# stujen/fiveEqSCM

Hardware: AMD Instinct MI355X
Metric: ensemble_member_timesteps_per_sec (higher is better)
Workload: dtype f64

## Files before the change

fiveeqscm_amd/csrc/fiveeq_member.hpp:

```cpp
#pragma once

namespace fiveeq {

template <typename V>
__device__ __forceinline__ V gas_forcing(const KGas<typename Lane<V>::S>& kg, const V Cg) {
    using S = typename Lane<V>::S;
    const auto pos = fe_gt0(Cg);
    V Fg = kg.f2 * (Cg - kg.C0);
    if constexpr (Lane<V>::W == 1) {
        if (kg.f1 != S(0)) Fg = pos ? fe_fma(kg.f1, fe_log(pos ? Cg * kg.inv_C0 : S(1)), Fg) : Fg;
        if (kg.f3 != S(0)) Fg = fe_fma(kg.f3, (pos ? fe_sqrt(pos ? Cg : S(1)) : S(0)) - kg.sqrtC0, Fg);
    } else {
        if (kg.f1 != S(0)) Fg = fe_sel(pos, fma3<V>(kg.f1, fe_log(fe_sel(pos, Cg * kg.inv_C0, (V)S(1))), Fg), Fg);
        if (kg.f3 != S(0)) Fg = fma3<V>(kg.f3, fe_sel(pos, fe_sqrt(fe_sel(pos, Cg, (V)S(1))), (V)S(0)) - kg.sqrtC0, Fg);
    }
    return Fg;
}

template <typename V, typename L, int g, bool INV, bool COMP = false>
__device__ __forceinline__ V gas_step(const KModel<typename Lane<V>::S>& km, const KGas<typename Lane<V>::S>& kg,
                                      const typename Lane<V>::S* __restrict__ drv, const V (&rr)[3 * L::G], const V T_old,
                                      V (&R)[L::SP], V (&out)[L::G], V (&cum)[L::G], V (&Rlo)[L::SP]) {
    using S = typename Lane<V>::S;
    static_assert(!INV || Lane<V>::W == 1, "the concentration-driven form has no packed instantiation");
    static_assert(!COMP || (!INV && sizeof(S) == 4), "the compensated form is an fp32 form of the emission-driven step");
    constexpr int P = L::pools(g);
    constexpr int o = L::off(g);
    V sumR = R[o];
#pragma unroll
    for (int i = 1; i < P; ++i) sumR += R[o + i];
    const V G_a = sumR * kg.inv_c;
    V G_u;
    if constexpr (INV) G_u = cum[g] - G_a;
    else G_u = drv[3 + g] - G_a;
    V iirf = fma3<V>(kg.ra, G_a, fma3<V>(rr[3 * g + 2], T_old, fma3<V>(rr[3 * g + 1], G_u, rr[3 * g])));
    iirf = fe_min(iirf, km.iirf_max);
    const V alpha = kg.g0 * fe_exp(iirf * kg.inv_g1);
    const V inv_alpha = fe_rcp(alpha);
    V em1[P];
#pragma unroll
    for (int i = 0; i < P; ++i) em1[i] = fe_expm1_neg(kg.ndt_over_tau[i] * inv_alpha);
    V E;
    if constexpr (INV) {
        V num = V(0), den = V(0);
#pragma unroll
        for (int i = 0; i < P; ++i) {
            num += fe_fma(R[o + i], em1[i], R[o + i]);
            den = fe_fma(kg.atc[i], em1[i], den);
        }
        E = (num - (drv[g] - kg.C0)) / (alpha * den);
        cum[g] = fe_fma(E, km.dt, cum[g]);
        out[g] = E;
    } else {
        E = (V)drv[g];
    }
    const V Ea = E * alpha;
    V sumN = (V)S(0);
#pragma unroll
    for (int i = 0; i < P; ++i) {
        const V Ri = R[o + i];
        V Rn;
        if constexpr (COMP) {
            const V y = fe_fma(em1[i], fma3<V>(-kg.atc[i], Ea, Ri), Rlo[o + i]);
            Rn = Ri + y;
            Rlo[o + i] = y - (Rn - Ri);
        } else {
            Rn = fe_fma(em1[i], fma3<V>(-kg.atc[i], Ea, Ri), Ri);
        }
        R[o + i] = Rn;
        sumN += Rn;
    }
    const V Cg = kg.C0 + sumN;
    if constexpr (!INV) out[g] = Cg;
    if constexpr (COMP) {
        const auto pos = fe_gt0(Cg);
        V Fg = kg.f2 * sumN;
        if (kg.f1 != S(0)) {
            const V x = sumN * kg.inv_C0;
            const V u = fe_sel(pos, (V)S(1) + x, (V)S(1));
            const V lg = fe_log(u) + (x - (u - (V)S(1)));
            Fg = fe_sel(pos, fma3<V>(kg.f1, lg, Fg), Fg);
        }
        if (kg.f3 != S(0)) {
            const V den = fe_sqrt(fe_sel(pos, Cg, (V)S(1))) + kg.sqrtC0;
            Fg = fma3<V>(kg.f3, fe_sel(pos, sumN * fe_rcp(den), (V)(-kg.sqrtC0)), Fg);
        }
        return Fg;
    } else {
        return gas_forcing<V>(kg, Cg);
    }
}

constexpr int MAX_FEXT = 4;
template <typename V, typename L, bool INV, bool COMP, bool FORC = false>
__device__ __forceinline__ void member_step(const KModel<typename Lane<V>::S>& km, const typename Lane<V>::S* __restrict__ drv,
                                            const V (&rr)[3 * L::G], const V (&qq)[2],
                                            V (&R)[L::SP], V (&S)[2], V (&out)[L::G], V& Tnew, V (&cum)[L::G],
                                            V (&Rlo)[L::SP], const V* fs = nullptr, const int fs_stride = 1,
                                            const typename Lane<V>::S* xr = nullptr, const int n_fext = 0) {
    static_assert(!FORC || (!INV && !COMP), "the forcing scales are carried by the plain forward form only");
    const V T_old = S[0] + S[1];
    V F = (V)drv[6];
    if constexpr (FORC) {
#pragma unroll
        for (int k = 0; k < MAX_FEXT; ++k)
            if (k < n_fext) F = fma3<V>(fs[(L::G + k) * fs_stride], xr[k], F);
    }
    asm volatile("" ::: "memory");
    const V F0 = gas_step<V, L, 0, INV, COMP>(km, km.gas[0], drv, rr, T_old, R, out, cum, Rlo);
    if constexpr (FORC) F = fe_fma(fs[0 * fs_stride], F0, F);
    else F += F0;
    if constexpr (L::G > 1) {
        asm volatile("" ::: "memory");
        const V F1 = gas_step<V, L, 1, INV, COMP>(km, km.gas[1], drv, rr, T_old, R, out, cum, Rlo);
        if constexpr (FORC) F = fe_fma(fs[1 * fs_stride], F1, F);
        else F += F1;
    }
    if constexpr (L::G > 2) {
        asm volatile("" ::: "memory");
        const V F2 = gas_step<V, L, 2, INV, COMP>(km, km.gas[2], drv, rr, T_old, R, out, cum, Rlo);
        if constexpr (FORC) F = fe_fma(fs[2 * fs_stride], F2, F);
        else F += F2;
    }
#pragma unroll
    for (int j = 0; j < 2; ++j) S[j] = fma3<V>(km.em1_d[j], fe_fma(-qq[j], F, S[j]), S[j]);
    Tnew = S[0] + S[1];
}
template <typename V, typename L, bool INV = false>
__device__ __forceinline__ void member_step(const KModel<typename Lane<V>::S>& km, const typename Lane<V>::S* __restrict__ drv,
                                            const V (&rr)[3 * L::G], const V (&qq)[2],
                                            V (&R)[L::SP], V (&S)[2], V (&out)[L::G], V& Tnew, V (&cum)[L::G]) {
    V no_Rlo[L::SP];
    member_step<V, L, INV, false>(km, drv, rr, qq, R, S, out, Tnew, cum, no_Rlo);
}
template <typename V, typename L>
__device__ __forceinline__ void member_step(const KModel<typename Lane<V>::S>& km, const typename Lane<V>::S* __restrict__ drv,
                                            const V (&rr)[3 * L::G], const V (&qq)[2],
                                            V (&R)[L::SP], V (&S)[2], V (&C)[L::G], V& Tnew) {
    V unused[L::G];
    member_step<V, L, false>(km, drv, rr, qq, R, S, C, Tnew, unused);
}

__device__ __forceinline__ void misfit_update(const double o, const double p, const double b, const double Tw, double& A,
                                              double& U, double& Vq) {
    A = A + b * Tw;
    const double d = Tw - o;
    const double pd = p * d;
    U = U + pd;
    Vq = Vq + pd * d;
}
__device__ __forceinline__ double lane_member(const double v, int) { return v; }
__device__ __forceinline__ double lane_member(const float v, int) { return (double)v; }
__device__ __forceinline__ double lane_member(const float2v v, int j) { return (double)(j == 0 ? v.x : v.y); }

template <typename T>
__device__ __forceinline__ void stage_model(KModel<T>* dst) {
    constexpr int NW = sizeof(KModel<T>) / sizeof(T);
    const T* src = (const T*)__builtin_amdgcn_kernarg_segment_ptr();
    for (int i = threadIdx.x; i < NW; i += FIVEEQ_BLOCK) reinterpret_cast<T*>(dst)[i] = src[i];
}

template <typename V>
__device__ __forceinline__ V load_lane(const typename Lane<V>::S* p) { return *reinterpret_cast<const V*>(p); }
__device__ __forceinline__ void store_lane(double* p, double v, bool) { *p = v; }
__device__ __forceinline__ void store_lane(float* p, float v, bool) { *p = v; }
__device__ __forceinline__ void store_lane(float* p, float2v v, bool full) {
    if (full) *reinterpret_cast<float2v*>(p) = v;
    else *p = v.x;
}
template <typename V, bool NT>
__device__ __forceinline__ V load_row(const typename Lane<V>::S* p) {
    if constexpr (NT) return __builtin_nontemporal_load(reinterpret_cast<const V*>(p));
    else return load_lane<V>(p);
}
template <bool NT, typename S, typename V>
__device__ __forceinline__ void store_row(S* p, V v, bool full) {
    if constexpr (!NT) store_lane(p, v, full);
    else if constexpr (sizeof(V) == sizeof(S)) __builtin_nontemporal_store(v, p);
    else {
        if (full) __builtin_nontemporal_store(v, reinterpret_cast<V*>(p));
        else __builtin_nontemporal_store(v.x, p);
    }
}

template <typename V>
__device__ __forceinline__ void misfit_step(const double* ob, const V Tn, double* acc, const int64_t mem_stride,
                                            const int64_t word_stride, const bool full) {
    const double o_t = ob[0], p_t = ob[1], b_t = ob[2];
    if (p_t != 0.0 || b_t != 0.0) {
#pragma unroll
        for (int j = 0; j < Lane<V>::W; ++j) {
            if (j == 0 || full) {
                double* a = acc + j * mem_stride;
                double A = a[0], U = a[word_stride], Vq = a[2 * word_stride];
                misfit_update(o_t, p_t, b_t, lane_member(Tn, j), A, U, Vq);
                a[0] = A;
                a[word_stride] = U;
                a[2 * word_stride] = Vq;
            }
        }
    }
}

enum Park { PARK_FIRST, PARK_LAST };
struct LaneSpan {
    int64_t m;
    bool active, full;
    int64_t mm;
};
template <int W, int BLOCK, Park PARK>
__device__ __forceinline__ LaneSpan lane_span(const int64_t n) {
    const int64_t m = ((int64_t)blockIdx.x * BLOCK + threadIdx.x) * W;
    const bool active = m < n;
    const bool full = m + (W - 1) < n;
    const int64_t mm = active ? m : (PARK == PARK_LAST ? ((n - 1) & ~(int64_t)(W - 1)) : 0);
    return LaneSpan{m, active, full, mm};
}

}
```

fiveeqscm_amd/csrc/fiveeq_step.hpp:

```cpp
#pragma once

namespace fiveeq {


#ifdef FIVEEQ_STEP_WAVES
#define FIVEEQ_STEP_ATTR __attribute__((amdgpu_waves_per_eu(FIVEEQ_STEP_WAVES, FIVEEQ_STEP_WAVES)))
#else
#define FIVEEQ_STEP_ATTR
#endif
template <typename T>
struct UniformRows {
    uint32_t mask;
    T val[3 * MAX_GAS + 2];
};
template <typename V, int P0, int P1, int P2, bool BINS, bool NT, bool MISFIT, bool FORC, bool UNI>
__device__ __forceinline__ void step_body(
    const typename Lane<V>::S* __restrict__ drive, const int n_steps, const int t,
    const int64_t n, const int64_t ld,
    const typename Lane<V>::S* __restrict__ r, const typename Lane<V>::S* __restrict__ q,
    typename Lane<V>::S* __restrict__ R, typename Lane<V>::S* __restrict__ S,
    typename Lane<V>::S* __restrict__ C_traj, typename Lane<V>::S* __restrict__ T_traj,
    const int n_rows, double* __restrict__ stats,
    unsigned short* __restrict__ bin_ring, const int ring_rows,
    const double hist_lo, const double hist_inv_w, const int n_bins,
    const double* __restrict__ obs, double* __restrict__ misfit,
    const typename Lane<V>::S* __restrict__ fscale,
    const typename Lane<V>::S* __restrict__ fext, const int n_fext,
    const UniformRows<typename Lane<V>::S>& uni) {
    using L = Layout<P0, P1, P2>;
    using T = typename Lane<V>::S;
    constexpr int W = Lane<V>::W;
    constexpr bool NTT = true;
    static_assert(!FORC || (!BINS && !NT), "the forcing scales: no histogram ring, default row policy");
    static_assert(!UNI || (!BINS && !MISFIT && !FORC), "the single-valued rows: the plain forward form only");
    __shared__ T drv[DRIVE_STRIDE];
    const auto [m, active, full, mm] = lane_span<W, FIVEEQ_STEP_BLOCK, PARK_LAST>(n);
    __shared__ KModel<T> km_s;
    constexpr int NW = sizeof(KModel<T>) / sizeof(T);
    static_assert(NW <= FIVEEQ_STEP_BLOCK, "model must stage in one pass");
    const T* kargs = (const T*)__builtin_amdgcn_kernarg_segment_ptr();
    T stage_v = T(0), drv_v = T(0);
    if (threadIdx.x < NW) stage_v = kargs[threadIdx.x];
    if (threadIdx.x < DRIVE_STRIDE) drv_v = drive[(int64_t)t * DRIVE_STRIDE + threadIdx.x];
    const KModel<T>& kmr = km_s;

    V rr[3 * L::G], qq[2], Rv[L::SP], Sv[2], Cv[L::G];
#pragma unroll
    for (int k = 0; k < L::SP; ++k) Rv[k] = load_row<V, NT>(R + k * ld + mm);
#pragma unroll
    for (int k = 0; k < 2; ++k) Sv[k] = load_row<V, NT>(S + k * ld + mm);
    if constexpr (UNI) {
#pragma unroll
        for (int k = 0; k < 3 * L::G; ++k) {
            if (uni.mask & (1u << k)) rr[k] = (V)uni.val[k];
            else rr[k] = load_row<V, NT>(r + k * ld + mm);
        }
#pragma unroll
        for (int k = 0; k < 2; ++k) {
            if (uni.mask & (1u << (3 * L::G + k))) qq[k] = (V)uni.val[3 * L::G + k];
            else qq[k] = load_row<V, NT>(q + k * ld + mm);
        }
    } else {
#pragma unroll
        for (int k = 0; k < 3 * L::G; ++k) rr[k] = load_row<V, NT>(r + k * ld + mm);
#pragma unroll
        for (int k = 0; k < 2; ++k) qq[k] = load_row<V, NT>(q + k * ld + mm);
    }
    V fs[FORC ? L::G + MAX_FEXT : 1];
    if constexpr (FORC) {
#pragma unroll
        for (int k = 0; k < L::G + MAX_FEXT; ++k) fs[k] = k < L::G + n_fext ? load_row<V, NT>(fscale + k * ld + mm) : (V)T(0);
    }

    if (threadIdx.x < NW) reinterpret_cast<T*>(&km_s)[threadIdx.x] = stage_v;
    if (threadIdx.x < DRIVE_STRIDE) drv[threadIdx.x] = drv_v;
    __syncthreads();

    V Tn = (V)T(0);
    if constexpr (FORC) {
        V no_cum[L::G], no_Rlo[L::SP];
        member_step<V, L, false, false, true>(kmr, drv, rr, qq, Rv, Sv, Cv, Tn, no_cum, no_Rlo, fs, 1,
                                              fext + (int64_t)t * MAX_FEXT, n_fext);
    } else {
        member_step<V, L>(kmr, drv, rr, qq, Rv, Sv, Cv, Tn);
    }
    if (active) {
#pragma unroll
        for (int k = 0; k < L::SP; ++k) store_row<NT>(R + k * ld + m, Rv[k], full);
#pragma unroll
        for (int k = 0; k < 2; ++k) store_row<NT>(S + k * ld + m, Sv[k], full);
        const int row = __builtin_amdgcn_readfirstlane((int)drv[7]);
        if (row >= 0 && row < n_rows) {
            if (C_traj != nullptr) {
                T* c = C_traj + (int64_t)row * L::G * ld + m;
#pragma unroll
                for (int g = 0; g < L::G; ++g) store_row<NTT>(c + g * ld, Cv[g], full);
            }
            if (T_traj != nullptr) store_row<NTT>(T_traj + (int64_t)row * ld + m, Tn, full);
        }
        if constexpr (MISFIT) misfit_step(obs + (int64_t)t * 4, Tn, misfit + m, 1, ld, full);
        if constexpr (BINS)
            store_bin(bin_ring + (int64_t)(t % ring_rows) * ld + m, make_rule(T(0), hist_lo, hist_inv_w, n_bins), Tn, full);
    }
    if (stats != nullptr) {
        const int64_t n_rec = (n + 63) >> 6;
        const int64_t wave = (int64_t)blockIdx.x * (FIVEEQ_STEP_BLOCK / 64) + (threadIdx.x >> 6);
        if constexpr (W == 1) {
            if (wave < n_rec) wave_stats(active, Tn, stats + (wave * n_steps + t) * 4);
        } else {
            if (2 * wave < n_rec)
                wave_stats(active, full, Tn, stats + (2 * wave * n_steps + t) * 4,
                           2 * wave + 1 < n_rec ? stats + ((2 * wave + 1) * n_steps + t) * 4 : nullptr);
        }
    }
}

template <typename V, int P0, int P1, int P2, bool BINS = false, bool NT = false, bool MISFIT = false, bool FORC = false>
__global__ __launch_bounds__(FIVEEQ_STEP_BLOCK) FIVEEQ_STEP_ATTR void step_kernel(
    const KModel<typename Lane<V>::S> km, const typename Lane<V>::S* __restrict__ drive, const int n_steps, const int t,
    const int64_t n, const int64_t ld,
    const typename Lane<V>::S* __restrict__ r, const typename Lane<V>::S* __restrict__ q,
    typename Lane<V>::S* __restrict__ R, typename Lane<V>::S* __restrict__ S,
    typename Lane<V>::S* __restrict__ C_traj ,
    typename Lane<V>::S* __restrict__ T_traj ,
    const int n_rows, double* __restrict__ stats ,
    unsigned short* __restrict__ bin_ring , const int ring_rows,
    const double hist_lo, const double hist_inv_w, const int n_bins,
    const double* __restrict__ obs , double* __restrict__ misfit ,
    const typename Lane<V>::S* __restrict__ fscale ,
    const typename Lane<V>::S* __restrict__ fext , const int n_fext) {
    step_body<V, P0, P1, P2, BINS, NT, MISFIT, FORC, false>(drive, n_steps, t, n, ld, r, q, R, S, C_traj, T_traj, n_rows, stats,
                                                            bin_ring, ring_rows, hist_lo, hist_inv_w, n_bins, obs, misfit, fscale,
                                                            fext, n_fext, UniformRows<typename Lane<V>::S>{});
}

template <typename V, int P0, int P1, int P2, bool NT = false>
__global__ __launch_bounds__(FIVEEQ_STEP_BLOCK) FIVEEQ_STEP_ATTR void step_uniform_kernel(
    const KModel<typename Lane<V>::S> km, const typename Lane<V>::S* __restrict__ drive, const int n_steps, const int t,
    const int64_t n, const int64_t ld,
    const typename Lane<V>::S* __restrict__ r, const typename Lane<V>::S* __restrict__ q,
    typename Lane<V>::S* __restrict__ R, typename Lane<V>::S* __restrict__ S,
    typename Lane<V>::S* __restrict__ C_traj ,
    typename Lane<V>::S* __restrict__ T_traj ,
    const int n_rows, double* __restrict__ stats ,
    const UniformRows<typename Lane<V>::S> uni) {
    step_body<V, P0, P1, P2, false, NT, false, false, true>(drive, n_steps, t, n, ld, r, q, R, S, C_traj, T_traj, n_rows, stats,
                                                            nullptr, 0, 0.0, 0.0, 0, nullptr, nullptr, nullptr, nullptr, 0, uni);
}

template <typename U>
__global__ __launch_bounds__(FIVEEQ_BLOCK) void uniform_rows_kernel(const int64_t n, const int64_t ld, const int n_r,
                                                                    const U* __restrict__ rows_r, const U* __restrict__ rows_q,
                                                                    unsigned int* __restrict__ differs, U* __restrict__ first) {
    const int row = blockIdx.y;
    const U* p = row < n_r ? rows_r + (int64_t)row * ld : rows_q + (int64_t)(row - n_r) * ld;
    const U v0 = p[0];
    U diff = 0;
    for (int64_t i = (int64_t)blockIdx.x * FIVEEQ_BLOCK + threadIdx.x; i < n; i += (int64_t)gridDim.x * FIVEEQ_BLOCK)
        diff |= p[i] ^ v0;
    if (__ballot(diff != 0) != 0 && (threadIdx.x & 63) == 0) atomicOr(differs, 1u << row);
    if (blockIdx.x == 0 && threadIdx.x == 0) first[row] = v0;
}

template <typename V, typename L>
struct ScenForc {
    static constexpr bool FS_LDS = false;
};
template <>
struct ScenForc<double, Layout<4, 1, 1>> {
    static constexpr bool FS_LDS = true;
};
template <typename V, int P0, int P1, int P2, bool NT = false, bool FORC = false>
__global__ __launch_bounds__(FIVEEQ_STEP_BLOCK) FIVEEQ_STEP_ATTR void step_scen_kernel(
    const KModel<typename Lane<V>::S> km, const typename Lane<V>::S* __restrict__ drive, const int n_steps, const int t,
    const int64_t n, const int64_t ld, const int n_scen,
    const typename Lane<V>::S* __restrict__ r, const typename Lane<V>::S* __restrict__ q,
    typename Lane<V>::S* __restrict__ R, typename Lane<V>::S* __restrict__ S,
    typename Lane<V>::S* __restrict__ C_traj, typename Lane<V>::S* __restrict__ T_traj,
    const int n_rows, double* __restrict__ stats,
    const typename Lane<V>::S* __restrict__ fscale ,
    const typename Lane<V>::S* __restrict__ fext , const int n_fext) {
    using L = Layout<P0, P1, P2>;
    using T = typename Lane<V>::S;
    constexpr int W = Lane<V>::W;
    constexpr bool NTT = true;
    static_assert(!FORC || !NT, "the forcing scales: default row policy");
    constexpr bool FS_LDS = FORC && ScenForc<V, L>::FS_LDS;
    const auto [m, active, full, mm] = lane_span<W, FIVEEQ_STEP_BLOCK, PARK_LAST>(n);
    __shared__ KModel<T> km_s;
    constexpr int NW = sizeof(KModel<T>) / sizeof(T);
    static_assert(NW <= FIVEEQ_STEP_BLOCK, "model must stage in one pass");
    const T* kargs = (const T*)__builtin_amdgcn_kernarg_segment_ptr();
    T stage_v = T(0);
    if (threadIdx.x < NW) stage_v = kargs[threadIdx.x];
    const KModel<T>& kmr = km_s;

    V rr[3 * L::G], qq[2], Rv[L::SP], Sv[2], Cv[L::G];
#pragma unroll
    for (int k = 0; k < 3 * L::G; ++k) rr[k] = load_row<V, NT>(r + k * ld + mm);
#pragma unroll
    for (int k = 0; k < 2; ++k) qq[k] = load_row<V, NT>(q + k * ld + mm);
    __shared__ V fs_s[FS_LDS ? (L::G + MAX_FEXT) * FIVEEQ_STEP_BLOCK : 1];
    V fs_r[FORC && !FS_LDS ? L::G + MAX_FEXT : 1];
    V* const fs = FS_LDS ? &fs_s[threadIdx.x] : fs_r;
    constexpr int FS_STRIDE = FS_LDS ? FIVEEQ_STEP_BLOCK : 1;
    if constexpr (FORC) {
#pragma unroll
        for (int k = 0; k < L::G + MAX_FEXT; ++k)
            fs[k * FS_STRIDE] = k < L::G + n_fext ? load_row<V, NT>(fscale + k * ld + mm) : (V)T(0);
    }
    if (threadIdx.x < NW) reinterpret_cast<T*>(&km_s)[threadIdx.x] = stage_v;
    __syncthreads();

    const int64_t n_rec = (n + 63) >> 6;
    const int64_t wave = (int64_t)blockIdx.x * (FIVEEQ_STEP_BLOCK / 64) + (threadIdx.x >> 6);
    const int64_t rec_stride = ((ld + 63) >> 6) * n_steps * 4;
    T* Rl = R + mm;
    T* Sl = S + mm;
#pragma unroll 1
    for (int sc = 0; sc < n_scen; ++sc, Rl += (int64_t)L::SP * ld, Sl += 2 * ld) {
#pragma unroll
        for (int k = 0; k < L::SP; ++k) Rv[k] = load_row<V, NT>(Rl + k * ld);
#pragma unroll
        for (int k = 0; k < 2; ++k) Sv[k] = load_row<V, NT>(Sl + k * ld);
        const T* d = drive + ((int64_t)sc * n_steps + t) * DRIVE_STRIDE;
        V Tn = (V)T(0);
        if constexpr (FORC) {
            V no_cum[L::G], no_Rlo[L::SP];
            member_step<V, L, false, false, true>(kmr, d, rr, qq, Rv, Sv, Cv, Tn, no_cum, no_Rlo, fs, FS_STRIDE,
                                                  fext + ((int64_t)sc * n_steps + t) * MAX_FEXT, n_fext);
        } else {
            member_step<V, L>(kmr, d, rr, qq, Rv, Sv, Cv, Tn);
        }
        if (active) {
#pragma unroll
            for (int k = 0; k < L::SP; ++k) store_row<NT>(Rl + k * ld, Rv[k], full);
#pragma unroll
            for (int k = 0; k < 2; ++k) store_row<NT>(Sl + k * ld, Sv[k], full);
            const int row = __builtin_amdgcn_readfirstlane((int)d[7]);
            if (row >= 0 && row < n_rows) {
                if (C_traj != nullptr) {
                    T* c = C_traj + ((int64_t)sc * n_rows + row) * L::G * ld + m;
#pragma unroll
                    for (int g = 0; g < L::G; ++g) store_row<NTT>(c + g * ld, Cv[g], full);
                }
                if (T_traj != nullptr) store_row<NTT>(T_traj + ((int64_t)sc * n_rows + row) * ld + m, Tn, full);
            }
        }
        if (stats != nullptr) {
            double* const st = stats + sc * rec_stride;
            if constexpr (W == 1) {
                if (wave < n_rec) wave_stats(active, Tn, st + (wave * n_steps + t) * 4);
            } else {
                if (2 * wave < n_rec)
                    wave_stats(active, full, Tn, st + (2 * wave * n_steps + t) * 4,
                               2 * wave + 1 < n_rec ? st + ((2 * wave + 1) * n_steps + t) * 4 : nullptr);
            }
        }
    }
}

}
```

Before: 32.06 billion.

## Interleave per-gas loads and stores with gas steps in f64 step kernel

For double precision, the step kernel now reorders its row loads so each gas's pools, parameters and forcing scale are loaded grouped by gas. A hook in member_step stores each gas's updated pools and concentration trajectory right after that gas is computed, instead of storing everything at the end. The aim is to overlap memory traffic with the transcendental-heavy gas arithmetic and shorten register live ranges. Per-gas stores issued in the middle of the step may interact with the asm memory barriers and change how the compiler schedules the code.

```diff
diff --git a/fiveeqscm_amd/csrc/fiveeq_member.hpp b/fiveeqscm_amd/csrc/fiveeq_member.hpp
--- a/fiveeqscm_amd/csrc/fiveeq_member.hpp
+++ b/fiveeqscm_amd/csrc/fiveeq_member.hpp
@@ -92,12 +92,21 @@
 }
 
 constexpr int MAX_FEXT = 4;
-template <typename V, typename L, bool INV, bool COMP, bool FORC = false>
+template <int g>
+struct GasTag {
+    static constexpr int value = g;
+};
+struct NoGasHook {
+    template <int g>
+    __device__ __forceinline__ void operator()(GasTag<g>) const {}
+};
+template <typename V, typename L, bool INV, bool COMP, bool FORC = false, typename Hook = NoGasHook>
 __device__ __forceinline__ void member_step(const KModel<typename Lane<V>::S>& km, const typename Lane<V>::S* __restrict__ drv,
                                             const V (&rr)[3 * L::G], const V (&qq)[2],
                                             V (&R)[L::SP], V (&S)[2], V (&out)[L::G], V& Tnew, V (&cum)[L::G],
                                             V (&Rlo)[L::SP], const V* fs = nullptr, const int fs_stride = 1,
-                                            const typename Lane<V>::S* xr = nullptr, const int n_fext = 0) {
+                                            const typename Lane<V>::S* xr = nullptr, const int n_fext = 0,
+                                            const Hook after_gas = Hook{}) {
     static_assert(!FORC || (!INV && !COMP), "the forcing scales are carried by the plain forward form only");
     const V T_old = S[0] + S[1];
     V F = (V)drv[6];
@@ -110,17 +119,20 @@
     const V F0 = gas_step<V, L, 0, INV, COMP>(km, km.gas[0], drv, rr, T_old, R, out, cum, Rlo);
     if constexpr (FORC) F = fe_fma(fs[0 * fs_stride], F0, F);
     else F += F0;
+    after_gas(GasTag<0>{});
     if constexpr (L::G > 1) {
         asm volatile("" ::: "memory");
         const V F1 = gas_step<V, L, 1, INV, COMP>(km, km.gas[1], drv, rr, T_old, R, out, cum, Rlo);
         if constexpr (FORC) F = fe_fma(fs[1 * fs_stride], F1, F);
         else F += F1;
+        after_gas(GasTag<1>{});
     }
     if constexpr (L::G > 2) {
         asm volatile("" ::: "memory");
         const V F2 = gas_step<V, L, 2, INV, COMP>(km, km.gas[2], drv, rr, T_old, R, out, cum, Rlo);
         if constexpr (FORC) F = fe_fma(fs[2 * fs_stride], F2, F);
         else F += F2;
+        after_gas(GasTag<2>{});
     }
 #pragma unroll
     for (int j = 0; j < 2; ++j) S[j] = fma3<V>(km.em1_d[j], fe_fma(-qq[j], F, S[j]), S[j]);
diff --git a/fiveeqscm_amd/csrc/fiveeq_step.hpp b/fiveeqscm_amd/csrc/fiveeq_step.hpp
--- a/fiveeqscm_amd/csrc/fiveeq_step.hpp
+++ b/fiveeqscm_amd/csrc/fiveeq_step.hpp
@@ -31,10 +31,13 @@
     using T = typename Lane<V>::S;
     constexpr int W = Lane<V>::W;
     constexpr bool NTT = true;
+    constexpr bool SPREAD = sizeof(T) == 8;
     static_assert(!FORC || (!BINS && !NT), "the forcing scales: no histogram ring, default row policy");
     static_assert(!UNI || (!BINS && !MISFIT && !FORC), "the single-valued rows: the plain forward form only");
     __shared__ T drv[DRIVE_STRIDE];
-    const auto [m, active, full, mm] = lane_span<W, FIVEEQ_STEP_BLOCK, PARK_LAST>(n);
+    const LaneSpan span = lane_span<W, FIVEEQ_STEP_BLOCK, PARK_LAST>(n);
+    const int64_t m = span.m, mm = span.mm;
+    const bool active = span.active, full = span.full;
     __shared__ KModel<T> km_s;
     constexpr int NW = sizeof(KModel<T>) / sizeof(T);
     static_assert(NW <= FIVEEQ_STEP_BLOCK, "model must stage in one pass");
@@ -45,53 +48,76 @@
     const KModel<T>& kmr = km_s;
 
     V rr[3 * L::G], qq[2], Rv[L::SP], Sv[2], Cv[L::G];
-#pragma unroll
-    for (int k = 0; k < L::SP; ++k) Rv[k] = load_row<V, NT>(R + k * ld + mm);
-#pragma unroll
-    for (int k = 0; k < 2; ++k) Sv[k] = load_row<V, NT>(S + k * ld + mm);
-    if constexpr (UNI) {
-#pragma unroll
-        for (int k = 0; k < 3 * L::G; ++k) {
-            if (uni.mask & (1u << k)) rr[k] = (V)uni.val[k];
-            else rr[k] = load_row<V, NT>(r + k * ld + mm);
-        }
-#pragma unroll
-        for (int k = 0; k < 2; ++k) {
-            if (uni.mask & (1u << (3 * L::G + k))) qq[k] = (V)uni.val[3 * L::G + k];
-            else qq[k] = load_row<V, NT>(q + k * ld + mm);
-        }
+    V fs[FORC ? L::G + MAX_FEXT : 1];
+    const auto par_row = [&](const T* __restrict__ rows, const int k, const int bit) -> V {
+        if constexpr (UNI) {
+            if (uni.mask & (1u << bit)) return (V)uni.val[bit];
+        }
+        return load_row<V, NT>(rows + k * ld + mm);
+    };
+    if constexpr (SPREAD) {
+#pragma unroll
+        for (int k = 0; k < 2; ++k) Sv[k] = load_row<V, NT>(S + k * ld + mm);
+        if constexpr (FORC) {
+#pragma unroll
+            for (int k = L::G; k < L::G + MAX_FEXT; ++k) fs[k] = k < L::G + n_fext ? load_row<V, NT>(fscale + k * ld + mm) : (V)T(0);
+        }
+#pragma unroll
+        for (int g = 0; g < L::G; ++g) {
+#pragma unroll
+            for (int i = 0; i < L::pools(g); ++i) Rv[L::off(g) + i] = load_row<V, NT>(R + (L::off(g) + i) * ld + mm);
+#pragma unroll
+            for (int k = 3 * g; k < 3 * g + 3; ++k) rr[k] = par_row(r, k, k);
+            if constexpr (FORC) fs[g] = load_row<V, NT>(fscale + g * ld + mm);
+        }
+#pragma unroll
+        for (int k = 0; k < 2; ++k) qq[k] = par_row(q, k, 3 * L::G + k);
     } else {
 #pragma unroll
-        for (int k = 0; k < 3 * L::G; ++k) rr[k] = load_row<V, NT>(r + k * ld + mm);
-#pragma unroll
-        for (int k = 0; k < 2; ++k) qq[k] = load_row<V, NT>(q + k * ld + mm);
-    }
-    V fs[FORC ? L::G + MAX_FEXT : 1];
-    if constexpr (FORC) {
-#pragma unroll
-        for (int k = 0; k < L::G + MAX_FEXT; ++k) fs[k] = k < L::G + n_fext ? load_row<V, NT>(fscale + k * ld + mm) : (V)T(0);
+        for (int k = 0; k < L::SP; ++k) Rv[k] = load_row<V, NT>(R + k * ld + mm);
+#pragma unroll
+        for (int k = 0; k < 2; ++k) Sv[k] = load_row<V, NT>(S + k * ld + mm);
+#pragma unroll
+        for (int k = 0; k < 3 * L::G; ++k) rr[k] = par_row(r, k, k);
+#pragma unroll
+        for (int k = 0; k < 2; ++k) qq[k] = par_row(q, k, 3 * L::G + k);
+        if constexpr (FORC) {
+#pragma unroll
+            for (int k = 0; k < L::G + MAX_FEXT; ++k) fs[k] = k < L::G + n_fext ? load_row<V, NT>(fscale + k * ld + mm) : (V)T(0);
+        }
     }
 
     if (threadIdx.x < NW) reinterpret_cast<T*>(&km_s)[threadIdx.x] = stage_v;
     if (threadIdx.x < DRIVE_STRIDE) drv[threadIdx.x] = drv_v;
     __syncthreads();
 
+    const int row = __builtin_amdgcn_readfirstlane((int)drv[7]);
+    const bool stored = row >= 0 && row < n_rows;
+    const auto store_gas = [&](auto gas) {
+        constexpr int g = decltype(gas)::value;
+        if (active) {
+#pragma unroll
+            for (int i = 0; i < L::pools(g); ++i) store_row<NT>(R + (L::off(g) + i) * ld + m, Rv[L::off(g) + i], full);
+            if (stored && C_traj != nullptr) store_row<NTT>(C_traj + ((int64_t)row * L::G + g) * ld + m, Cv[g], full);
+        }
+    };
     V Tn = (V)T(0);
-    if constexpr (FORC) {
-        V no_cum[L::G], no_Rlo[L::SP];
-        member_step<V, L, false, false, true>(kmr, drv, rr, qq, Rv, Sv, Cv, Tn, no_cum, no_Rlo, fs, 1,
-                                              fext + (int64_t)t * MAX_FEXT, n_fext);
-    } else {
-        member_step<V, L>(kmr, drv, rr, qq, Rv, Sv, Cv, Tn);
-    }
+    V no_cum[L::G], no_Rlo[L::SP];
+    if constexpr (SPREAD)
+        member_step<V, L, false, false, FORC>(kmr, drv, rr, qq, Rv, Sv, Cv, Tn, no_cum, no_Rlo, fs, 1,
+                                              FORC ? fext + (int64_t)t * MAX_FEXT : nullptr, n_fext, store_gas);
+    else
+        member_step<V, L, false, false, FORC>(kmr, drv, rr, qq, Rv, Sv, Cv, Tn, no_cum, no_Rlo, fs, 1,
+                                              FORC ? fext + (int64_t)t * MAX_FEXT : nullptr, n_fext);
     if (active) {
-#pragma unroll
-        for (int k = 0; k < L::SP; ++k) store_row<NT>(R + k * ld + m, Rv[k], full);
+        if constexpr (!SPREAD) {
+#pragma unroll
+            for (int k = 0; k < L::SP; ++k) store_row<NT>(R + k * ld + m, Rv[k], full);
+        }
 #pragma unroll
         for (int k = 0; k < 2; ++k) store_row<NT>(S + k * ld + m, Sv[k], full);
-        const int row = __builtin_amdgcn_readfirstlane((int)drv[7]);
-        if (row >= 0 && row < n_rows) {
-            if (C_traj != nullptr) {
+        if (stored) {
+            if (!SPREAD && C_traj != nullptr) {
                 T* c = C_traj + (int64_t)row * L::G * ld + m;
 #pragma unroll
                 for (int g = 0; g < L::G; ++g) store_row<NTT>(c + g * ld, Cv[g], full);
```

Result: faster. 32.43 billion, median of 6 (+1.1%).
